# JinfengX/PointCloudPDF

Measured on AMD Instinct MI355X. Metric: points/sec fwd+bwd (PT-v1 Seg50 + PDF U-decoder, 100k-pt scenes), higher is better.
Workload: dtype f32

## Files before the change

include/pdfops.h:

```cpp
#ifndef PDFOPS_H
#define PDFOPS_H

#ifdef __cplusplus
extern "C" {
#endif

#define PDF_OK 0
#define PDF_ERR_BAD_ARG (-1)
#define PDF_ERR_NSAMPLE (-2)
#define PDF_ERR_UNSUPPORTED (-3)

#define PDF_ABI_VERSION 7
int pdf_abi_version(void);
const char *pdf_build_info(void);
int pdf_dist_fma_mode(void);
#define PDF_MMA_F32 0
#define PDF_MMA_F16 1
#define PDF_MMA_BF16 2

int pdf_knn_query(int m, int nsample, const float *xyz, const float *new_xyz,
                  const int *offset, const int *new_offset, int b,
                  int *idx, float *dist2, void *stream);

long pdf_knn_workspace_bytes(int b, int n, int m);
// ... 69 lines not shown
                      const float *new_xyz, const int *idx, float *output, void *stream);
int pdf_group_backward(int m, int nsample, int c, int with_xyz, const float *grad_output, const int *idx,
                       float *grad_feat, void *stream);

int pdf_interpolation_weights(int n, int k, const float *dist2, float *weight, void *stream);

int pdf_pt_layer_supported(int nsample, int c);
long pdf_pt_layer_partial_floats(int n, int nsample, int c);
int pdf_pt_layer_forward(int n, int nsample, int c, const float *xq, const float *xk, const float *xv,
                         const float *p, const int *idx, const float *const *weights,
                         const float *const *bn_params, float *const *bn_buffers, int training, float eps,
                         float momentum, float *bn, float *saved, float *H, float *partial, float *out,
                         int storage_bf16, const int *order, void *stream);
int pdf_pt_layer_forward_m(int n, int nsample, int c, const float *xq, const float *xk, const float *xv,
                           const float *p, const int *idx, const float *const *weights,
                           const float *const *bn_params, float *const *bn_buffers, int training, float eps,
                           float momentum, float *bn, float *saved, float *H, float *partial, float *out,
                           int storage_bf16, const int *order, const double *moments, int *out_stat_rows, void *stream);

long pdf_pt_layer_bwd_partial_floats(int n, int nsample, int c);
long pdf_pt_layer_bwd_sums_floats(int c);
int pdf_pt_layer_backward(int n, int nsample, int c, const float *xq, const float *xk, const float *xv,
                          const float *p, const int *idx, const float *const *weights, const float *bn,
                          const float *saved, const float *H, const float *gout, float *gxq, float *gxk,
                          float *gxv, float *G2, float *G3, float *Wsm, float *GR, const int *inv_off, const int *inv_entry,
                          int entry_base, float *partial, float *sums, int storage_bf16, const int *order, const double *moments,
                          void *stream);

int pdf_bn_supported(int c);
long pdf_bn_partial_floats(long n, int c);
int pdf_bn_act_forward(long n, int c, const float *x, const float *res, const float *gamma, const float *beta,
                       float *running_mean, float *running_var, int training, float eps, float momentum, int relu,
                       float *coef, float *partial, float *y, void *stream);
int pdf_bn_act_backward(long n, int c, const float *gy, const float *x, const float *res, const float *coef,
                        int training, int relu, float *partial, float *sums, float *gx, float *gres, void *stream);
int pdf_bn_coef(long n, int c, const float *x, const float *gamma, const float *beta, float *running_mean,
                float *running_var, int training, float eps, float momentum, float *coef, float *partial, void *stream);
int pdf_bn_apply(long n, int c, const float *x, const float *res, const float *coef, int relu, float *y, void *stream);

long pdf_rowlin_partial_floats(long n, int o);
int pdf_rowlin_partial_rows(long n, int k, int o);
int pdf_rowlin_forward(long n, int k, int o, const float *x, long ldx, const float *w, int transpose_w,
                       const float *bias, const float *scale, const float *shift, int relu, float *y, long ldy,
                       int accumulate, float *partial, int mma_input, void *stream);
long pdf_rowlin_wgrad_ws_floats(long n, int k, int o, int ng);
int pdf_rowlin_wgrad(long n, int k, int o, const float *g, long ldg, const float *x, long ldx,
                     const float *scale, const float *shift, int relu, float *dw, float *db, float *ws, int mma_input, void *stream);
int pdf_bn_coef_from_partial(const float *partial, int rows, long n, int c, const float *gamma, const float *beta,
                             float *running_mean, float *running_var, float eps, float momentum, float *coef, void *stream);

int pdf_rowlin_multi(long n, int k, int o, int nin, int nout, const float *const *x, long ldx, const float *const *w,
                     int transpose_w, const float *const *bias, const float *scale, const float *shift, int relu,
                     float *const *y, long ldy, int accumulate, int mma_input, void *stream);
int pdf_rowlin_wgrad_multi(long n, int k, int o, int ng, const float *const *g, long ldg, const float *x, long ldx,
                           const float *scale, const float *shift, int relu, float *const *dw, float *const *db, float *ws, int mma_input, void *stream);
int pdf_rowlin_wgrad_group(long n, int k, int o, int ng, const float *const *g, long ldg, const float *const *x, long ldx,
                           const float *const *scale, const float *const *shift, const int *relu, float *const *dw,
                           float *const *db, float *ws, int mma_input, void *stream);

int pdf_kpconv_supported(int kp, int cin);
int pdf_kpconv_gather(int n, int m, int kp, int cin, const float *query, const float *support, const int *neighbors, const float *x,
                      const float *k_points, float extent, float *weighted, void *stream);
int pdf_kpconv_scatter(int n, int m, int kp, int cin, const float *query, const float *support, const int *neighbors,
                       const float *grad_weighted, const float *k_points, float extent, float *grad_x, void *stream);
int pdf_rowlin_dgrad_bstats(long n, int k, int o, int nin, const float *const *x, long ldx, const float *const *w, float *y, long ldy,
                            const float *bx, long ldb, const float *bcoef, int brelu, float *partial, int *partial_rows,
                            int mma_input, void *stream);
int pdf_rowlin_forward_bn(long n, int k, int o, const float *x, long ldx, const float *w, const float *bias, const float *scale,
                          const float *shift, int relu, float *y, long ldy, float *partial, const float *gamma, const float *beta,
                          float *running_mean, float *running_var, float eps, float momentum, float *coef, int mma_input, void *stream);
int pdf_bn_act_backward_presummed(long n, int c, const float *gy, const float *x, const float *coef, int training, int relu,
                                  const float *partial, int partial_rows, float *sums, float *gx, void *stream);

int pdf_bn_coef_eval_or_partial(const float *partial, int rows, long n, int c, const float *gamma, const float *beta,
                                float *running_mean, float *running_var, int training, float eps, float momentum,
                                float *coef, void *stream);
int pdf_block_pre_forward(long n, int c, void *const *p, int training, float eps, float momentum, int mma_input, void *stream);
int pdf_block_pre_backward(long n, int c, void *const *p, int training, int mma_input, void *stream);
int pdf_block_post_forward(long n, int c, void *const *p, int training, float eps, float momentum, int mma_input, void *stream);
int pdf_block_post_backward(long n, int c, void *const *p, int training, int mma_input, void *stream);
int pdf_bottleneck_forward(long n, int nsample, int c, void *const *p, int training, float eps, float momentum, int storage_bf16, int mma_input, void *stream);
int pdf_bottleneck_backward(long n, int nsample, int c, void *const *p, int training, int entry_base, int storage_bf16, int mma_input, void *stream);
int pdf_linbn_forward(long n, int k, int o, void *const *p, int training, int relu, float eps, float momentum, int mma_input, void *stream);
int pdf_linbn_backward(long n, int k, int o, void *const *p, int training, int relu, int mma_input, void *stream);

int pdf_rowlin_forward_roww(long n, int k, int o, const float *x, long ldx, const float *w, int transpose_w, float *y, long ldy,
                            int accumulate, const float *roww, long rws, int mma_input, void *stream);
int pdf_rowlin_wgrad_roww(long n, int k, int o, const float *g, long ldg, const float *x, long ldx, float *dw, const float *roww,
                          long rws, float *ws, int mma_input, void *stream);
int pdf_bn_bwd_sums(long n, int c, const float *gy, const float *x, const float *coef, int relu, float *partial, float *sums,
                    void *stream);

int pdf_td_supported(int nsample, int cin, int cout);
int pdf_td_tables(long m, int b, const float *p_src, const float *p_new, const int *idx, const int *new_offset, float *rel4, float *Z,
                  float *scene_sums, long n, const int *inv_off, const int *inv_entry, int entry_base,
                  void *stream);
long pdf_td_gram_floats(int cin);
long pdf_td_fwd_scratch_floats(long n, int cin);
long pdf_td_bwd_scratch_floats(long m, int cin, int cout);
int pdf_td_forward(long n, long m, int cin, int cout, void *const *p, int training, float eps, float momentum, int mma_input, void *stream);
int pdf_td_backward(long n, long m, int cin, int cout, void *const *p, int entry_base, int mma_input, void *stream);

int pdf_seg_sum_rows(long n, int c, const float *src, const int *inv_off, const int *inv_entry, int entry_base, float scale, float *out,
                     void *stream);
int pdf_seg_sum_rows_own(long n, int c, int nsample, const float *src, const int *inv_off, const int *inv_entry, int entry_base, float scale,
                         const int *order, float *out, float *out_own, void *stream);
// ... 184 lines not shown
```

pointcloudpdf_amd/_native.py:

```python
import ctypes
import os
import threading

import torch

_HERE = os.path.dirname(os.path.abspath(__file__))
DIST_FMA = int(os.environ.get("PDFOPS_DIST_FMA", "0") or 0)
if DIST_FMA not in (0, 1, 2):
    raise RuntimeError(f"PDFOPS_DIST_FMA={DIST_FMA}: expected 0 (as written), 1 or 2 (csrc/pdfops_common.h)")


def library_path(dist_fma=0):
    return os.path.join(_HERE, "lib", "libpdfops.so" if not dist_fma else f"libpdfops_fma{int(dist_fma)}.so")


LIB_PATH = library_path(DIST_FMA)
ABI_VERSION = 7

c_int = ctypes.c_int
c_long = ctypes.c_long
c_void_p = ctypes.c_void_p
c_float = ctypes.c_float
c_double = ctypes.c_double

# ... 598 lines not shown
        self.CopySeg = CopySeg
        lib.pdf_stage_copy.restype = c_int
        lib.pdf_stage_copy.argtypes = [c_int, c_void_p, c_void_p]
        lib.pdf_scene_morton_keys.restype = c_int
        lib.pdf_scene_morton_keys.argtypes = [c_long, c_int, c_void_p, c_void_p, c_void_p, c_void_p, c_void_p]
        lib.pdf_sgd_chunk.restype = c_int
        lib.pdf_sgd_chunk.argtypes = []
        lib.pdf_sgd_step.restype = c_int
        lib.pdf_sgd_step.argtypes = [c_int, c_void_p, c_void_p, ctypes.c_float, ctypes.c_float, ctypes.c_float, c_void_p, c_void_p]
        lib.pdf_grad_unscale.restype = c_int
        lib.pdf_grad_unscale.argtypes = [c_int, c_void_p, c_void_p, c_void_p, c_void_p, c_void_p]
        lib.pdf_scaler_update.restype = c_int
        lib.pdf_scaler_update.argtypes = [c_void_p, c_void_p, c_void_p, c_void_p, ctypes.c_float, ctypes.c_float, c_int, c_void_p]
        lib.pdf_adam_step.restype = c_int
        lib.pdf_adam_step.argtypes = [c_int, c_int, c_void_p, c_void_p, ctypes.c_double, ctypes.c_double, ctypes.c_double, ctypes.c_double,
                                      ctypes.c_double, c_int, c_void_p, c_void_p]
        lib.pdf_adam_grad_unscale.restype = c_int
        lib.pdf_adam_grad_unscale.argtypes = [c_int, c_void_p, c_void_p, c_void_p, c_void_p, c_void_p]
        lib.pdf_linbn_forward.restype = c_int
        lib.pdf_linbn_forward.argtypes = [c_long, c_int, c_int, c_void_p, c_int, c_int, ctypes.c_float, ctypes.c_float, c_int, c_void_p]
        lib.pdf_linbn_backward.restype = c_int
        lib.pdf_linbn_backward.argtypes = [c_long, c_int, c_int, c_void_p, c_int, c_int, c_int, c_void_p]
        lib.pdf_bottleneck_forward.restype = c_int
        lib.pdf_bottleneck_forward.argtypes = [c_long, c_int, c_int, c_void_p, c_int, ctypes.c_float, ctypes.c_float, c_int, c_int, c_void_p]
        lib.pdf_bottleneck_backward.restype = c_int
        lib.pdf_bottleneck_backward.argtypes = [c_long, c_int, c_int, c_void_p, c_int, c_int, c_int, c_int, c_void_p]
        for nm in ("pre_backward", "post_backward"):
            f = getattr(lib, "pdf_block_" + nm)
            f.restype = c_int
            f.argtypes = [c_long, c_int, c_void_p, c_int, c_int, c_void_p]
        lib.pdf_rowlin_multi.restype = c_int
        lib.pdf_rowlin_multi.argtypes = [c_long, c_int, c_int, c_int, c_int, c_void_p, c_long, c_void_p, c_int, c_void_p, c_void_p, c_void_p,
                                         c_int, c_void_p, c_long, c_int, c_int, c_void_p]
        lib.pdf_kpconv_supported.restype = c_int
        lib.pdf_kpconv_supported.argtypes = [c_int, c_int]
        for nm in ("pdf_kpconv_gather", "pdf_kpconv_scatter"):
            f = getattr(lib, nm)
            f.restype = c_int
            f.argtypes = [c_int, c_int, c_int, c_int, c_void_p, c_void_p, c_void_p, c_void_p, c_void_p, ctypes.c_float, c_void_p, c_void_p]
        lib.pdf_rowlin_wgrad_group.restype = c_int
        lib.pdf_rowlin_wgrad_group.argtypes = [c_long, c_int, c_int, c_int, c_void_p, c_long, c_void_p, c_long, c_void_p, c_void_p, c_void_p,
                                               c_void_p, c_void_p, c_void_p, c_int, c_void_p]
        lib.pdf_rowlin_wgrad_multi.restype = c_int
        lib.pdf_rowlin_wgrad_multi.argtypes = [c_long, c_int, c_int, c_int, c_void_p, c_long, c_void_p, c_long, c_void_p, c_void_p, c_int,
                                               c_void_p, c_void_p, c_void_p, c_int, c_void_p]
        lib.pdf_rowlin_wgrad_ws_floats.restype = c_long
        lib.pdf_rowlin_wgrad_ws_floats.argtypes = [c_long, c_int, c_int, c_int]
        lib.pdf_rowlin_dgrad_bstats.restype = c_int
        lib.pdf_rowlin_dgrad_bstats.argtypes = [c_long, c_int, c_int, c_int, c_void_p, c_long, c_void_p, c_void_p, c_long, c_void_p, c_long,
                                                c_void_p, c_int, c_void_p, ctypes.POINTER(c_int), c_int, c_void_p]
        lib.pdf_bn_act_backward_presummed.restype = c_int
        lib.pdf_bn_act_backward_presummed.argtypes = [c_long, c_int, c_void_p, c_void_p, c_void_p, c_int, c_int, c_void_p, c_int, c_void_p,
                                                      c_void_p, c_void_p]
        lib.pdf_rowlin_partial_floats.restype = c_long
        lib.pdf_rowlin_partial_floats.argtypes = [c_long, c_int]
        lib.pdf_rowlin_partial_rows.restype = c_int
        lib.pdf_rowlin_partial_rows.argtypes = [c_long, c_int, c_int]
        lib.pdf_rowlin_forward.restype = c_int
        lib.pdf_rowlin_forward.argtypes = [c_long, c_int, c_int, c_void_p, c_long, c_void_p, c_int, c_void_p, c_void_p, c_void_p,
                                           c_int, c_void_p, c_long, c_int, c_void_p, c_int, c_void_p]
        lib.pdf_rowlin_wgrad.restype = c_int
        lib.pdf_rowlin_wgrad.argtypes = [c_long, c_int, c_int, c_void_p, c_long, c_void_p, c_long, c_void_p, c_void_p, c_int,
                                         c_void_p, c_void_p, c_void_p, c_int, c_void_p]
        lib.pdf_bn_coef_from_partial.restype = c_int
        lib.pdf_bn_coef_from_partial.argtypes = [c_void_p, c_int, c_long, c_int, c_void_p, c_void_p, c_void_p, c_void_p,
                                                 ctypes.c_float, ctypes.c_float, c_void_p, c_void_p]
        lib.pdf_bn_coef.restype = c_int
        lib.pdf_bn_coef.argtypes = [c_long, c_int, c_void_p, c_void_p, c_void_p, c_void_p, c_void_p, c_int, ctypes.c_float,
                                    ctypes.c_float, c_void_p, c_void_p, c_void_p]
        lib.pdf_bn_apply.restype = c_int
        lib.pdf_bn_apply.argtypes = [c_long, c_int, c_void_p, c_void_p, c_void_p, c_int, c_void_p, c_void_p]
        lib.pdf_bn_supported.restype = c_int
        lib.pdf_bn_supported.argtypes = [c_int]
        lib.pdf_bn_partial_floats.restype = c_long
        lib.pdf_bn_partial_floats.argtypes = [c_long, c_int]
        lib.pdf_bn_act_forward.restype = c_int
        lib.pdf_bn_act_forward.argtypes = [c_long, c_int] + [c_void_p] * 6 + [c_int, ctypes.c_float, ctypes.c_float, c_int] + [c_void_p] * 4
        lib.pdf_bn_act_backward.restype = c_int
        lib.pdf_bn_act_backward.argtypes = [c_long, c_int] + [c_void_p] * 4 + [c_int, c_int] + [c_void_p] * 5
        lib.pdf_pt_layer_supported.restype = c_int
        lib.pdf_pt_layer_supported.argtypes = [c_int, c_int]
        for fn in (lib.pdf_pt_layer_partial_floats, lib.pdf_pt_layer_bwd_partial_floats):
            fn.restype = c_long
            fn.argtypes = [c_int, c_int, c_int]
        lib.pdf_pt_layer_bwd_sums_floats.restype = c_long
        lib.pdf_pt_layer_bwd_sums_floats.argtypes = [c_int]
        lib.pdf_pt_layer_forward.restype = c_int
        lib.pdf_pt_layer_forward.argtypes = [c_int, c_int, c_int] + [c_void_p] * 8 + [c_int, ctypes.c_float, ctypes.c_float] + [c_void_p] * 5 + [c_int, c_void_p, c_void_p]
        lib.pdf_knn_grid_build.restype = c_int
        lib.pdf_knn_grid_build.argtypes = [c_int, c_void_p, c_void_p, c_int, c_void_p, c_long, c_void_p]
        lib.pdf_knn_query_grid.restype = c_int
        lib.pdf_knn_query_grid.argtypes = [c_int, c_int, c_int, c_void_p, c_void_p, c_void_p, c_void_p, c_int, c_void_p, c_void_p, c_void_p, c_long, c_void_p]
        lib.pdf_pt_layer_backward.restype = c_int
        lib.pdf_pt_layer_backward.argtypes = [c_int, c_int, c_int] + [c_void_p] * 19 + [c_int] + [c_void_p] * 2 + [c_int, c_void_p, c_void_p, c_void_p]
        self.fps_mode = os.environ.get("PDFOPS_FPS", "bucketed")
        self.knn_mode = os.environ.get("PDFOPS_KNN", "grid")
        lib.pdf_knn_workspace_bytes.restype = c_long
        lib.pdf_knn_workspace_bytes.argtypes = [c_int, c_int, c_int]
        lib.pdf_graph_forest_workspace_bytes.restype = c_long
        lib.pdf_region_grow_list_points.restype = c_long
        lib.pdf_region_grow_list_points.argtypes = []
        lib.pdf_graph_forest_workspace_bytes.argtypes = [c_long, c_long, c_long]
        lib.pdf_knn_grid_supported.restype = c_int
        lib.pdf_knn_grid_supported.argtypes = [c_int]
        lib.pdf_knn_query_ws.restype = c_int
        lib.pdf_knn_query_ws.argtypes = [c_int, c_int, c_int] + [c_void_p] * 4 + [c_int] + [c_void_p] * 3 + [c_long, c_void_p]
# ... 965 lines not shown
```

pointcloudpdf_amd/csrc/rowlin.hip:

```cpp
#include "pdfops_common.h"
#include <cstdlib>

namespace rl {

typedef float f32x16 __attribute__((ext_vector_type(16)));
constexpr int BM = 128, BN = 64, BK = 32, LDT = 33;

struct FwdArgs {
    long N;
    int K, O;
    const float *X; long ldx;
    const float *W; long wso, wsk;
    const float *bias;
    const float *scale, *shift;
    int relu;
    float *Y; long ldy;
    int accumulate;
    float *partial;
};

template <bool PRE, bool STATS>
__global__ __launch_bounds__(256) void k_rowlin(FwdArgs a) {
    __shared__ float xs[BM * LDT];
    __shared__ float ws[BN * LDT];
// ... 112 lines not shown
            g[u] = (r < re && ov) ? a.G[r * a.ldg + oc] : 0.f;
            float v = 0.f;
            if (r < re && cv) {
                v = a.X[r * a.ldx + cc];
                if (PRE) { v = v * sc + sh; if (a.relu) v = fmaxf(v, 0.f); }
            }
            x[u] = v;
        }
#pragma unroll
        for (int u = 0; u < 4; ++u) {
            acc = __builtin_amdgcn_mfma_f32_32x32x2f32(g[u], x[u], acc, 0, 0, 0);
            gsum += g[u];
        }
    }
    __shared__ float comb[4][1024 + 32];
#pragma unroll
    for (int r = 0; r < 16; ++r) {
        const int i = (r & 3) + 8 * (r >> 2) + 4 * (lane >> 5);
        comb[wave][i * 32 + ch] = acc[r];
    }
    gsum += __shfl_xor(gsum, 32, 64);
    if (lane < 32) comb[wave][1024 + ch] = gsum;
    __syncthreads();
    const size_t sidx = blockIdx.x, nsl = gridDim.x;
    float *slab = a.slab + ((size_t)blockIdx.y * nsl + sidx) * 1024;
#pragma unroll
    for (int e = threadIdx.x; e < 1024; e += 256) slab[e] = ((comb[0][e] + comb[1][e]) + comb[2][e]) + comb[3][e];
    if (a.db && c0 == 0 && threadIdx.x < 32)
        a.bslab[((size_t)(o0 / 32) * nsl + sidx) * 32 + threadIdx.x] =
            ((comb[0][1024 + threadIdx.x] + comb[1][1024 + threadIdx.x]) + comb[2][1024 + threadIdx.x]) + comb[3][1024 + threadIdx.x];
}

}

namespace rl2 {
int try_forward(long n, int k, int o, int nin, int nout, const float *const *x, long ldx, const float *const *w, int transpose_w,
                const float *const *bias, const float *scale, const float *shift, int relu, float *const *y, long ldy,
                int accumulate, float *partial, int mma, hipStream_t s, const float *roww = nullptr, long rws = 0, const float *bx = nullptr,
                long ldb = 0, const float *bcoef = nullptr, int brelu = 0, int *partial_rows = nullptr, long ldw = 0, void *handoff = nullptr);
long stats_rows_floats(long n, int o);
int try_wgrad(long n, int k, int o, int ng, const float *const *g, long ldg, const float *x, long ldx, const float *scale,
              const float *shift, int relu, float *const *dw, float *const *db, float *ws, int mma, hipStream_t s, const float *roww = nullptr, long rws = 0);
long wgrad_ws_floats(long n, int k, int o, int ng);
constexpr int WG_MAXG = 5;
struct RArgs {
    const float *slab, *bslab;
    float *dW[WG_MAXG], *db[WG_MAXG];
    int B, tiles_k, tiles, otiles, split, K, O;
};
int try_wgrad_group(long n, int k, int o, int ng, const float *const *g, long ldg, const float *const *x, long ldx, const float *const *scale,
                    const float *const *shift, const int *relu, float *const *dw, float *const *db, float *ws, int mma, hipStream_t s);
void launch_slab_reduce(const RArgs &a, int ng, bool any_bias, hipStream_t s);
int stats_rows(long n);
}

static inline void tiled_wg_plan(long n, int k, int o, int *blocks_oc, long *split, long *rows_per_block) {
    *blocks_oc = ((o + 31) / 32) * ((k + 31) / 32);
    long sp = (2048 + *blocks_oc - 1) / *blocks_oc;
    const long max_split = (n + 255) / 256;
    if (sp > max_split) sp = max_split;
    if (sp < 1) sp = 1;
    *rows_per_block = ((n + sp - 1) / sp + 31) / 32 * 32;
    *split = (n + *rows_per_block - 1) / *rows_per_block;
}

static inline bool rowlin_streams(int k, int o) {
    return (k == 32 || k == 64 || k == 128 || k == 256 || k == 512) && o % 16 == 0 && getenv("PDFOPS_ROWLIN_TILED") == nullptr;
}

extern "C" int pdf_rowlin_partial_rows(long n, int k, int o) {
    return rowlin_streams(k, o) ? rl2::stats_rows(n) : (int)((n + rl::BM - 1) / rl::BM);
}
extern "C" long pdf_rowlin_partial_floats(long n, int o) {
    const long a = (n + rl::BM - 1) / rl::BM * 2 * (long)o, b = rl2::stats_rows_floats(n, o);
    return (a > b ? a : b) + (long)PDF_HO_FLOATS;
}

extern "C" int pdf_rowlin_forward(long n, int k, int o, const float *x, long ldx, const float *w, int transpose_w,
                                  const float *bias, const float *scale, const float *shift, int relu, float *y, long ldy,
                                  int accumulate, float *partial, int mma_input, void *stream) {
    if (mma_input < 0 || mma_input > 2) return PDF_ERR_BAD_ARG;
    if (n < 1 || k < 1 || o < 1 || !x || !w || !y || ldx < k || ldy < o) return PDF_ERR_BAD_ARG;
    if (rowlin_streams(k, o)) {
        if (rl2::try_forward(n, k, o, 1, 1, &x, ldx, &w, transpose_w, &bias, scale, shift, relu, &y, ldy, accumulate, partial,
                             mma_input, static_cast<hipStream_t>(stream)))
            return pdf_launch_status();
        if (partial) return PDF_ERR_BAD_ARG;
    }
    if (!transpose_w && !partial && !scale && k == 1024 && rowlin_streams(512, o) && !(ldx & 3) && !(ldy & 3)) {
        const float *xs[2] = {x, x + 512}, *ws[2] = {w, w + 512};
        if (rl2::try_forward(n, 512, o, 2, 1, xs, ldx, ws, 0, &bias, nullptr, nullptr, 0, &y, ldy, accumulate, nullptr, mma_input, static_cast<hipStream_t>(stream),
                             nullptr, 0, nullptr, 0, nullptr, 0, nullptr, k))
            return pdf_launch_status();
    }
    rl::FwdArgs a;
    a.N = n; a.K = k; a.O = o; a.X = x; a.ldx = ldx; a.W = w;
    a.wso = transpose_w ? 1 : k; a.wsk = transpose_w ? o : 1;
    a.bias = bias; a.scale = scale; a.shift = shift; a.relu = relu; a.Y = y; a.ldy = ldy; a.accumulate = accumulate;
    a.partial = partial;
    const dim3 grid((unsigned)((n + rl::BM - 1) / rl::BM), (unsigned)((o + rl::BN - 1) / rl::BN));
    hipStream_t s = static_cast<hipStream_t>(stream);
    const bool pre = scale != nullptr, stats = partial != nullptr;
    if (pre && stats) rl::k_rowlin<true, true><<<grid, 256, 0, s>>>(a);
    else if (pre) rl::k_rowlin<true, false><<<grid, 256, 0, s>>>(a);
    else if (stats) rl::k_rowlin<false, true><<<grid, 256, 0, s>>>(a);
    else rl::k_rowlin<false, false><<<grid, 256, 0, s>>>(a);
    return pdf_launch_status();
}

extern "C" long pdf_rowlin_wgrad_ws_floats(long n, int k, int o, int ng) {
    if (n < 1 || k < 1 || o < 1 || ng < 1) return 0;
    int blocks_oc; long split, rpb;
    tiled_wg_plan(n, k, o, &blocks_oc, &split, &rpb);
    const long tiled = (long)blocks_oc * split * 4 * 1024 + (long)((o + 31) / 32) * split * 4 * 32;
    const long streaming = rowlin_streams(k, o) ? rl2::wgrad_ws_floats(n, k, o, ng) : 0;
    return tiled > streaming ? tiled : streaming;
}

extern "C" int pdf_bn_coef_from_partial(const float *partial, int rows, long n, int c, const float *gamma, const float *beta,
                                        float *running_mean, float *running_var, float eps, float momentum, float *coef, void *stream);

extern "C" int pdf_rowlin_forward_bn(long n, int k, int o, const float *x, long ldx, const float *w, const float *bias, const float *scale,
                                     const float *shift, int relu, float *y, long ldy, float *partial, const float *gamma, const float *beta,
                                     float *running_mean, float *running_var, float eps, float momentum, float *coef, int mma_input, void *stream) {
// ... 125 lines not shown
```

pointcloudpdf_amd/csrc/rowlin2_impl.h:

```cpp
#pragma once
#include "pdfops_common.h"
#include <algorithm>
#include <cstdlib>

namespace rl2 {

typedef float f32x4 __attribute__((ext_vector_type(4)));

typedef _Float16 h16x4 __attribute__((ext_vector_type(4)));
typedef __bf16 b16x4 __attribute__((ext_vector_type(4)));
typedef short s16x4 __attribute__((ext_vector_type(4)));
template <int MP> struct Mma;
template <> struct Mma<0> {
    typedef f32x4 frag;
    static __device__ __forceinline__ frag cvt(f32x4 v) { return v; }
};
template <> struct Mma<1> {
    typedef h16x4 frag;
    static __device__ __forceinline__ frag cvt(f32x4 v) { return __builtin_convertvector(v, h16x4); }
    static __device__ __forceinline__ f32x4 mma(frag a, frag b, f32x4 acc) { return __builtin_amdgcn_mfma_f32_16x16x16f16(a, b, acc, 0, 0, 0); }
};
template <> struct Mma<2> {
    typedef s16x4 frag;
    static __device__ __forceinline__ frag cvt(f32x4 v) { return __builtin_bit_cast(s16x4, __builtin_convertvector(v, b16x4)); }
// ... 126 lines not shown
                            for (int ob = 0; ob < NOB; ++ob)
                                acc[ob] = __builtin_amdgcn_mfma_f32_16x16x4f32(Wr[in][ob][j][c], x4[c], acc[ob], 0, 0, 0);
                    } else {
                        const wfrag xh = Mma<MP>::cvt(x4);
#pragma unroll
                        for (int ob = 0; ob < NOB; ++ob) acc[ob] = Mma<MP>::mma(Wr[in][ob][j], xh, acc[ob]);
                    }
                }
            }
        }
#pragma unroll
        for (int ob = 0; ob < NOB; ++ob) {
            f32x4 v = acc[ob];
            if (a.roww) v *= a.roww[(valid ? n : 0) * a.rws];
            v += bias4[ob];
            float *dst = a.Y[outi[ob]] + (valid ? n : 0) * a.ldy + colb[ob] + 4 * kq;
            if (a.accumulate && valid) v += *reinterpret_cast<const f32x4 *>(dst);
            if (valid) *reinterpret_cast<f32x4 *>(dst) = v;
            if (ST == 1 && valid) { s4[ob] += v; ss4[ob] += v * v; }
            if (ST == 2) {
                const f32x4 x4 = *reinterpret_cast<const f32x4 *>(a.bx + (valid ? n : 0) * a.ldb + colb[ob] + 4 * kq);
                const f32x4 sc = *reinterpret_cast<const f32x4 *>(&bco[0][ob * 16 + 4 * kq]);
                const f32x4 sh = *reinterpret_cast<const f32x4 *>(&bco[ST == 2 ? 1 : 0][ob * 16 + 4 * kq]);
                const f32x4 mu = *reinterpret_cast<const f32x4 *>(&bco[ST == 2 ? 2 : 0][ob * 16 + 4 * kq]);
                const f32x4 pre = x4 * sc + sh;
                f32x4 gm;
#pragma unroll
                for (int c = 0; c < 4; ++c) gm[c] = (valid && (!a.brelu || pre[c] > 0.f)) ? v[c] : 0.f;
                s4[ob] += gm;
                ss4[ob] += gm * (x4 - mu);
            }
        }
    }
    if (STATS) {
        __shared__ float red[4][2][NOB * 16];
#pragma unroll
        for (int ob = 0; ob < NOB; ++ob)
#pragma unroll
            for (int r = 0; r < 4; ++r) {
                float s = s4[ob][r], ss = ss4[ob][r];
#pragma unroll
                for (int m = 1; m < 16; m <<= 1) { s += __shfl_xor(s, m, 64); ss += __shfl_xor(ss, m, 64); }
                if (li == 0) { red[wave][0][ob * 16 + 4 * kq + r] = s; red[wave][1][ob * 16 + 4 * kq + r] = ss; }
            }
        __syncthreads();
        const int t = threadIdx.x;
        if (t < NOB * 16) {
            float *row = a.partial + (size_t)blockIdx.x * 2 * a.O;
            row[gcol0 + t] = red[0][0][t] + red[1][0][t] + red[2][0][t] + red[3][0][t];
            const float ss = red[0][1][t] + red[1][1][t] + red[2][1][t] + red[3][1][t];
            row[a.O + gcol0 + t] = ST == 2 ? ss * a.bcoef[3 * (long)a.O + gcol0 + t] : ss;
        }
    }
}

constexpr int WG_MAXG = 5;
struct WArgs {
    long N;
    int K, O;
    const float *G[WG_MAXG]; long ldg;
    const float *X; long ldx;
    const float *scale, *shift; int relu;
    int per_z; const float *Xz[WG_MAXG]; const float *scalez[WG_MAXG], *shiftz[WG_MAXG]; int reluz[WG_MAXG];
    float *dW[WG_MAXG], *db[WG_MAXG];
    long rows_per_block;
    const float *roww; long rws;
    float *slab;
    float *bslab;
};

template <int VW> struct Vec;
template <> struct Vec<2> { typedef float type __attribute__((ext_vector_type(2))); };
template <> struct Vec<4> { typedef float type __attribute__((ext_vector_type(4))); };

template <int VW, bool PRE, bool RW, int MP>
__global__ __launch_bounds__(256) void k_wg(WArgs a) {
    typedef typename Vec<VW>::type vec;
    constexpr int B = 16 * VW;
    __shared__ float red[4][B * B];
    __shared__ float redb[4][B];
    const int lane = threadIdx.x & 63, wave = threadIdx.x >> 6;
    const int li = lane & 15, nq = lane >> 4;
    const int nkb = a.K / B;
    const int ob = (blockIdx.y / nkb) * B, kb = (blockIdx.y % nkb) * B;
    const float *G = a.G[blockIdx.z];
    const float *X = (PRE && a.per_z) ? a.Xz[blockIdx.z] : a.X;
    vec sc, sh;
    bool relu = a.relu != 0;
    if (PRE) {
        const float *scp = a.per_z ? a.scalez[blockIdx.z] : a.scale, *shp = a.per_z ? a.shiftz[blockIdx.z] : a.shift;
        if (a.per_z) relu = scp != nullptr && a.reluz[blockIdx.z] != 0;
        if (scp) {
            sc = *reinterpret_cast<const vec *>(scp + kb + VW * li);
            sh = *reinterpret_cast<const vec *>(shp + kb + VW * li);
        } else {
#pragma unroll
            for (int c = 0; c < VW; ++c) { sc[c] = 1.f; sh[c] = 0.f; }
        }
    }
    const float relu_lo = relu ? 0.f : -INFINITY;
    f32x4 acc[VW][VW];
    float gsum[VW];
#pragma unroll
    for (int c = 0; c < VW; ++c) {
        gsum[c] = 0.f;
#pragma unroll
// ... 151 lines not shown
static inline bool aligned16(const void *p) { return (reinterpret_cast<uintptr_t>(p) & 15) == 0; }

template <int K, int NOB, int NIN, int MP>
static int launch_fwd(const FwdArgs &a, int nslabs, hipStream_t s) {
    const bool pre = a.scale != nullptr, stats = a.partial != nullptr, bst = stats && a.bx != nullptr;
    static const int total = [] { const char *v = getenv("PDFOPS_RL_BLOCKS"); const int x = v ? atoi(v) : 0; return x > 0 ? x : 512; }();
    int gx = fwd_row_blocks(a.N);
    if (!stats || bst) gx = std::max(1, std::min(gx, std::max(8, total / std::max(nslabs, 1))));
    const dim3 grid((unsigned)gx, (unsigned)nslabs);
    if (bst) {
        k_fwd<K, NOB, NIN, false, 2, MP><<<grid, 256, 0, s>>>(a);
    } else if (NIN == 1 && stats) {
        if (pre) k_fwd<K, NOB, 1, true, 1, MP><<<grid, 256, 0, s>>>(a);
        else k_fwd<K, NOB, 1, false, 1, MP><<<grid, 256, 0, s>>>(a);
    } else {
        if (pre) k_fwd<K, NOB, NIN, true, 0, MP><<<grid, 256, 0, s>>>(a);
        else k_fwd<K, NOB, NIN, false, 0, MP><<<grid, 256, 0, s>>>(a);
    }
    return gx;
}

#ifdef RL2_MAIN_TU
long stats_rows_floats(long n, int o) { return (long)fwd_row_blocks(n) * 2 * o; }
#endif

template <int MP>
int try_forward_mp(long n, int k, int o, int nin, int nout, const float *const *x, long ldx, const float *const *w, int transpose_w,
                   const float *const *bias, const float *scale, const float *shift, int relu, float *const *y, long ldy,
                   int accumulate, float *partial, hipStream_t s, const float *roww, long rws, const float *bx, long ldb, const float *bcoef,
                   int brelu, int *partial_rows, long ldw, void *handoff) {
    if (nin < 1 || nout < 1 || (nin > 1 && nout > 1) || nin > 3 || nout > 3) return 0;
    if (nin == 2 && (scale || bx)) return 0;
    if (partial && !bx && (nin != 1 || nout != 1)) return 0;
    if (bx && (!partial || nout != 1 || scale || !bcoef || (ldb & 3) || !aligned16(bx) || !aligned16(bcoef))) return 0;
    if ((ldx & 3) || (ldy & 3) || (o & 15)) return 0;
    for (int i = 0; i < (nin > 1 ? nin : nout); ++i) if (!aligned16(w[i])) return 0;
    if (scale && (!aligned16(scale) || !aligned16(shift))) return 0;
    for (int i = 0; i < nin; ++i) if (!aligned16(x[i])) return 0;
    for (int i = 0; i < nout; ++i) if (!aligned16(y[i])) return 0;
    FwdArgs a;
    a.N = n; a.O = o; a.ldx = ldx; a.ldy = ldy; a.scale = scale; a.shift = shift; a.relu = relu; a.accumulate = accumulate;
    a.partial = partial; a.roww = roww; a.rws = rws;
    a.bx = bx; a.ldb = ldb; a.bcoef = bcoef; a.brelu = brelu;
    a.ho_gran = static_cast<unsigned long long *>(handoff);
    a.ho_sync = handoff ? reinterpret_cast<unsigned *>(a.ho_gran + 2 * (size_t)o) : nullptr;
    a.wso = transpose_w ? 1 : (ldw ? ldw : k); a.wsk = transpose_w ? o : 1;
    for (int i = 0; i < 3; ++i) {
        a.X[i] = i < nin ? x[i] : nullptr;
        a.W[i] = i < (nin > 1 ? nin : nout) ? w[i] : nullptr;
        a.bias[i] = (bias && i < nout) ? bias[i] : nullptr;
        a.Y[i] = i < nout ? y[i] : nullptr;
    }
    const int cols = o * nout;
#define PDF_RL2(K_, NOB_, NIN_) do { if (cols % (NOB_ * 16) == 0) { \
        const int r_ = launch_fwd<K_, NOB_, NIN_, MP>(a, cols / (NOB_ * 16), s); \
        if (partial_rows) *partial_rows = r_; \
        return 1; } } while (0)
    if (nin == 1) {
        switch (k) {
        case 32: if (!partial) PDF_RL2(32, 6, 1); PDF_RL2(32, 2, 1); PDF_RL2(32, 1, 1); break;
        case 64: PDF_RL2(64, 4, 1); PDF_RL2(64, 1, 1); break;
        case 128: if (!bx) PDF_RL2(128, 4, 1); else PDF_RL2(128, 2, 1); PDF_RL2(128, 1, 1); break;
        case 256: PDF_RL2(256, 2, 1); PDF_RL2(256, 1, 1); break;
        case 512: PDF_RL2(512, 1, 1); break;
        default: break;
        }
    } else if (nin == 2) {
        if (k == 512) PDF_RL2(512, 1, 2);
    } else if (nin == 3) {
        switch (k) {
        case 32: PDF_RL2(32, 2, 3); break;
        case 64: PDF_RL2(64, 2, 3); break;
        case 128: PDF_RL2(128, 1, 3); break;
        case 256: PDF_RL2(256, 1, 3); break;
        default: break;
        }
    }
#undef PDF_RL2
    return 0;
}

template <int MP>
int try_wgrad_mp(long n, int k, int o, int ng, const float *const *g, long ldg, const float *x, long ldx, const float *scale,
                 const float *shift, int relu, float *const *dw, float *const *db, float *ws, hipStream_t s, const float *roww, long rws) {
    if (ng < 1 || ng > 3 || !ws) return 0;
    const WgPlan p = wg_plan(n, k, o, ng);
    const int vw = p.vw;
    if (!vw) return 0;
    if ((ldg % vw) || (ldx % vw) || !aligned16(x)) return 0;
    if (scale && (!aligned16(scale) || !aligned16(shift))) return 0;
    for (int i = 0; i < ng; ++i) if (!aligned16(g[i])) return 0;
    WArgs a;
    a.N = n; a.K = k; a.O = o; a.ldg = ldg; a.X = x; a.ldx = ldx; a.scale = scale; a.shift = shift; a.relu = relu; a.roww = roww; a.rws = rws;
    a.per_z = 0;
    bool any_bias = false;
    for (int i = 0; i < WG_MAXG; ++i) {
        a.G[i] = i < ng ? g[i] : nullptr; a.dW[i] = i < ng ? dw[i] : nullptr; a.db[i] = (db && i < ng) ? db[i] : nullptr;
        a.Xz[i] = nullptr; a.scalez[i] = a.shiftz[i] = nullptr; a.reluz[i] = 0;
        any_bias = any_bias || a.db[i] != nullptr;
    }
    const int b = p.b;
    a.rows_per_block = p.rows_per_block;
    a.slab = ws;
    a.bslab = ws + (size_t)p.nblk * p.split * b * b;
    const dim3 grid((unsigned)p.split, (unsigned)((o / b) * (k / b)), (unsigned)ng);
#define PDF_WG(VW_) do { \
        if (roww) { if (scale) k_wg<VW_, true, true, MP><<<grid, 256, 0, s>>>(a); else k_wg<VW_, false, true, MP><<<grid, 256, 0, s>>>(a); } \
        else      { if (scale) k_wg<VW_, true, false, MP><<<grid, 256, 0, s>>>(a); else k_wg<VW_, false, false, MP><<<grid, 256, 0, s>>>(a); } } while (0)
    if (vw == 4) PDF_WG(4); else PDF_WG(2);
#undef PDF_WG
    RArgs r;
    r.slab = a.slab; r.bslab = a.bslab; r.B = b; r.tiles_k = k / b; r.tiles = (o / b) * (k / b); r.otiles = o / b; r.split = (int)p.split; r.K = k; r.O = o;
    for (int i = 0; i < WG_MAXG; ++i) { r.dW[i] = a.dW[i]; r.db[i] = a.db[i]; }
    launch_slab_reduce(r, ng, any_bias, s);
    return 1;
}

template <int MP>
int try_wgrad_group_mp(long n, int k, int o, int ng, const float *const *g, long ldg, const float *const *x, long ldx,
                       const float *const *scale, const float *const *shift, const int *relu, float *const *dw, float *const *db,
                       float *ws, hipStream_t s) {
    if (ng < 1 || ng > WG_MAXG || !ws) return 0;
    const WgPlan p = wg_plan(n, k, o, ng);
    const int vw = p.vw;
    if (!vw) return 0;
    if ((ldg % vw) || (ldx % vw)) return 0;
    for (int i = 0; i < ng; ++i) {
        if (!aligned16(g[i]) || !aligned16(x[i])) return 0;
        if (scale[i] && (!aligned16(scale[i]) || !aligned16(shift[i]))) return 0;
    }
    WArgs a;
    a.N = n; a.K = k; a.O = o; a.ldg = ldg; a.X = nullptr; a.ldx = ldx; a.scale = a.shift = nullptr; a.relu = 0; a.roww = nullptr; a.rws = 0;
    a.per_z = 1;
    bool any_bias = false;
    for (int i = 0; i < WG_MAXG; ++i) {
        const bool on = i < ng;
        a.G[i] = on ? g[i] : nullptr; a.Xz[i] = on ? x[i] : nullptr;
        a.scalez[i] = on ? scale[i] : nullptr; a.shiftz[i] = on ? shift[i] : nullptr; a.reluz[i] = on ? relu[i] : 0;
        a.dW[i] = on ? dw[i] : nullptr; a.db[i] = (on && db) ? db[i] : nullptr;
        any_bias = any_bias || a.db[i] != nullptr;
    }
    const int b = p.b;
    a.rows_per_block = p.rows_per_block;
    a.slab = ws;
    a.bslab = ws + (size_t)p.nblk * p.split * b * b;
    const dim3 grid((unsigned)p.split, (unsigned)((o / b) * (k / b)), (unsigned)ng);
    if (vw == 4) k_wg<4, true, false, MP><<<grid, 256, 0, s>>>(a); else k_wg<2, true, false, MP><<<grid, 256, 0, s>>>(a);
    RArgs r;
    r.slab = a.slab; r.bslab = a.bslab; r.B = b; r.tiles_k = k / b; r.tiles = (o / b) * (k / b); r.otiles = o / b; r.split = (int)p.split; r.K = k; r.O = o;
    for (int i = 0; i < WG_MAXG; ++i) { r.dW[i] = a.dW[i]; r.db[i] = a.db[i]; }
    launch_slab_reduce(r, ng, any_bias, s);
    return 1;
}

#ifdef RL2_MAIN_TU
int stats_rows(long n) { return fwd_row_blocks(n); }
#endif

}
```

Baseline: 13.49 million.

## Add LDS-tiled MFMA forward kernel for multi-input/multi-output row linears

Adds a new forward kernel that stages 64-row by 64-K chunks of X (and transposed W for the 3-input case) in shared memory, with register prefetch of the next chunk. It is used for K in {128, 256, 512} with (nin=1, nout=3) or (nin=3, nout=1), and includes optional pre-scale/ReLU and fused BN-backward stats. The aim is to reuse each X tile across several output column tiles instead of streaming it from global memory per column block. A grid-size threshold chooses a narrow or wide column-block layout. It costs extra LDS traffic and barriers, and it is enabled by default with an env opt-out.

After: 13.71 million (median of 6 runs). 1.6% higher.

```diff
diff --git a/include/pdfops.h b/include/pdfops.h
--- a/include/pdfops.h
+++ b/include/pdfops.h
@@ -145,6 +145,7 @@
 int pdf_rowlin_multi(long n, int k, int o, int nin, int nout, const float *const *x, long ldx, const float *const *w,
                      int transpose_w, const float *const *bias, const float *scale, const float *shift, int relu,
                      float *const *y, long ldy, int accumulate, int mma_input, void *stream);
+int pdf_rowlin_tiled_covers(long n, int k, int nin, int nout, int bstats);
 int pdf_rowlin_wgrad_multi(long n, int k, int o, int ng, const float *const *g, long ldg, const float *x, long ldx,
                            const float *scale, const float *shift, int relu, float *const *dw, float *const *db, float *ws, int mma_input, void *stream);
 int pdf_rowlin_wgrad_group(long n, int k, int o, int ng, const float *const *g, long ldg, const float *const *x, long ldx,
diff --git a/pointcloudpdf_amd/_native.py b/pointcloudpdf_amd/_native.py
--- a/pointcloudpdf_amd/_native.py
+++ b/pointcloudpdf_amd/_native.py
@@ -674,6 +674,8 @@
         lib.pdf_bn_act_backward_presummed.restype = c_int
         lib.pdf_bn_act_backward_presummed.argtypes = [c_long, c_int, c_void_p, c_void_p, c_void_p, c_int, c_int, c_void_p, c_int, c_void_p,
                                                       c_void_p, c_void_p]
+        lib.pdf_rowlin_tiled_covers.restype = c_int
+        lib.pdf_rowlin_tiled_covers.argtypes = [c_long, c_int, c_int, c_int, c_int]
         lib.pdf_rowlin_partial_floats.restype = c_long
         lib.pdf_rowlin_partial_floats.argtypes = [c_long, c_int]
         lib.pdf_rowlin_partial_rows.restype = c_int
diff --git a/pointcloudpdf_amd/csrc/rowlin.hip b/pointcloudpdf_amd/csrc/rowlin.hip
--- a/pointcloudpdf_amd/csrc/rowlin.hip
+++ b/pointcloudpdf_amd/csrc/rowlin.hip
@@ -188,6 +188,7 @@
                     const float *const *shift, const int *relu, float *const *dw, float *const *db, float *ws, int mma, hipStream_t s);
 void launch_slab_reduce(const RArgs &a, int ng, bool any_bias, hipStream_t s);
 int stats_rows(long n);
+int tiled_covers_probe(long n, int k, int nin, int nout, int bstats);
 }
 
 static inline void tiled_wg_plan(long n, int k, int o, int *blocks_oc, long *split, long *rows_per_block) {
@@ -206,6 +207,9 @@
 
 extern "C" int pdf_rowlin_partial_rows(long n, int k, int o) {
     return rowlin_streams(k, o) ? rl2::stats_rows(n) : (int)((n + rl::BM - 1) / rl::BM);
+}
+extern "C" int pdf_rowlin_tiled_covers(long n, int k, int nin, int nout, int bstats) {
+    return rowlin_streams(k, k) ? rl2::tiled_covers_probe(n, k, nin, nout, bstats) : 0;
 }
 extern "C" long pdf_rowlin_partial_floats(long n, int o) {
     const long a = (n + rl::BM - 1) / rl::BM * 2 * (long)o, b = rl2::stats_rows_floats(n, o);
diff --git a/pointcloudpdf_amd/csrc/rowlin2_impl.h b/pointcloudpdf_amd/csrc/rowlin2_impl.h
--- a/pointcloudpdf_amd/csrc/rowlin2_impl.h
+++ b/pointcloudpdf_amd/csrc/rowlin2_impl.h
@@ -202,6 +202,192 @@
             row[a.O + gcol0 + t] = ST == 2 ? ss * a.bcoef[3 * (long)a.O + gcol0 + t] : ss;
         }
     }
+}
+
+constexpr int TL_ROWS = 64, TL_KC = 64, TL_LD = TL_KC + 4;
+
+template <int K, int WR, int NIN, bool PRE, int ST, int MP>
+__global__ __launch_bounds__(256) void k_fwd_tiled(FwdArgs a) {
+    typedef typename Mma<MP>::frag wfrag;
+    constexpr bool TW = NIN > 1;
+    constexpr int WC = 4 / WR, RT = 4 / WR;
+    constexpr int CB = 16 * WC, WLD = CB + 4;
+    constexpr int NCH = K / TL_KC, NS = NIN * NCH, NJ = TL_KC / 16;
+    constexpr int CPR = CB / 4, RPP = 256 / CPR, NWP = TL_KC / RPP;
+    __shared__ __attribute__((aligned(16))) float xs[TL_ROWS * TL_LD];
+    __shared__ __attribute__((aligned(16))) float wsm[TW ? TL_KC * WLD : 4];
+    const int lane = threadIdx.x & 63, wave = threadIdx.x >> 6;
+    const int li = lane & 15, kq = lane >> 4;
+    const int wr = wave / WC, wc = wave % WC;
+    const long row0 = (long)blockIdx.x * TL_ROWS;
+    const int gcol0 = blockIdx.y * CB;
+    const int outi = (gcol0 + wc * 16) / a.O, colb = gcol0 + wc * 16 - outi * a.O;
+    const int sx_c = 4 * (threadIdx.x & 15), sx_r = threadIdx.x >> 4;
+    const int sw_c = 4 * (threadIdx.x % CPR), sw_r = threadIdx.x / CPR;
+    long xoff[4];
+#pragma unroll
+    for (int i = 0; i < 4; ++i) { const long n = row0 + sx_r + 16 * i; xoff[i] = (n < a.N ? n : 0) * a.ldx + sx_c; }
+    const float *wrow = nullptr;
+    if (!TW) wrow = (outi == 0 ? a.W[0] : (outi == 1 ? a.W[1] : a.W[2])) + (long)(colb + li) * a.wso + 4 * kq;
+    const float relu_lo = a.relu ? 0.f : -INFINITY;
+    f32x4 xpf[4], scpf, shpf, wpf[TW ? NWP : NJ], wcur[TW ? 1 : NJ];
+    auto prefetch = [&](int s) {
+        const int in = s / NCH, kc0 = (s - in * NCH) * TL_KC;
+        const float *X = in == 0 ? a.X[0] : (in == 1 ? a.X[1] : a.X[2]);
+#pragma unroll
+        for (int i = 0; i < 4; ++i) xpf[i] = *reinterpret_cast<const f32x4 *>(X + xoff[i] + kc0);
+        if (PRE) {
+            scpf = *reinterpret_cast<const f32x4 *>(a.scale + kc0 + sx_c);
+            shpf = *reinterpret_cast<const f32x4 *>(a.shift + kc0 + sx_c);
+        }
+        if (TW) {
+            const float *W = in == 0 ? a.W[0] : (in == 1 ? a.W[1] : a.W[2]);
+#pragma unroll
+            for (int i = 0; i < NWP; ++i) wpf[i] = *reinterpret_cast<const f32x4 *>(W + (long)(kc0 + sw_r + RPP * i) * a.wsk + gcol0 + sw_c);
+        } else {
+#pragma unroll
+            for (int j = 0; j < NJ; ++j) wpf[j] = *reinterpret_cast<const f32x4 *>(wrow + kc0 + 16 * j);
+        }
+    };
+    f32x4 acc[RT];
+#pragma unroll
+    for (int t = 0; t < RT; ++t) acc[t] = f32x4{0.f, 0.f, 0.f, 0.f};
+    prefetch(0);
+#pragma unroll 1
+    for (int s = 0; s < NS; ++s) {
+        __syncthreads();
+#pragma unroll
+        for (int i = 0; i < 4; ++i) {
+            f32x4 x4 = xpf[i];
+            if (PRE) {
+                x4 = x4 * scpf + shpf;
+#pragma unroll
+                for (int c = 0; c < 4; ++c) x4[c] = fmaxf(x4[c], relu_lo);
+            }
+            *reinterpret_cast<f32x4 *>(&xs[(sx_r + 16 * i) * TL_LD + sx_c]) = x4;
+        }
+        if (TW) {
+#pragma unroll
+            for (int i = 0; i < NWP; ++i) *reinterpret_cast<f32x4 *>(&wsm[TW ? (sw_r + RPP * i) * WLD + sw_c : 0]) = wpf[i];
+        } else {
+#pragma unroll
+            for (int j = 0; j < NJ; ++j) wcur[TW ? 0 : j] = wpf[j];
+        }
+        __syncthreads();
+        if (s + 1 < NS) prefetch(s + 1);
+#pragma unroll
+        for (int j = 0; j < NJ; ++j) {
+            f32x4 a4, x4[RT];
+            if (TW) {
+#pragma unroll
+                for (int c = 0; c < 4; ++c) a4[c] = wsm[TW ? (16 * j + 4 * kq + c) * WLD + wc * 16 + li : 0];
+            } else {
+                a4 = wcur[TW ? 0 : j];
+            }
+#pragma unroll
+            for (int t = 0; t < RT; ++t) x4[t] = *reinterpret_cast<const f32x4 *>(&xs[(16 * (wr * RT + t) + li) * TL_LD + 16 * j + 4 * kq]);
+            if constexpr (MP == 0) {
+#pragma unroll
+                for (int c = 0; c < 4; ++c)
+#pragma unroll
+                    for (int t = 0; t < RT; ++t) acc[t] = __builtin_amdgcn_mfma_f32_16x16x4f32(a4[c], x4[t][c], acc[t], 0, 0, 0);
+            } else {
+                const wfrag ah = Mma<MP>::cvt(a4);
+#pragma unroll
+                for (int t = 0; t < RT; ++t) acc[t] = Mma<MP>::mma(ah, Mma<MP>::cvt(x4[t]), acc[t]);
+            }
+        }
+    }
+    const float *b = NIN > 1 ? a.bias[0] : (outi == 0 ? a.bias[0] : (outi == 1 ? a.bias[1] : a.bias[2]));
+    float *Y = outi == 0 ? a.Y[0] : (outi == 1 ? a.Y[1] : a.Y[2]);
+    const int col = colb + 4 * kq;
+    f32x4 bias4 = f32x4{0.f, 0.f, 0.f, 0.f};
+    if (b) bias4 = *reinterpret_cast<const f32x4 *>(b + col);
+    f32x4 bsc, bsh, bmu, s4 = f32x4{0.f, 0.f, 0.f, 0.f}, ss4 = f32x4{0.f, 0.f, 0.f, 0.f};
+    if (ST == 2) {
+        bsc = *reinterpret_cast<const f32x4 *>(a.bcoef + col);
+        bsh = *reinterpret_cast<const f32x4 *>(a.bcoef + (long)a.O + col);
+        bmu = *reinterpret_cast<const f32x4 *>(a.bcoef + 2 * (long)a.O + col);
+    }
+#pragma unroll
+    for (int t = 0; t < RT; ++t) {
+        const long n = row0 + 16 * (wr * RT + t) + li;
+        const bool valid = n < a.N;
+        const long nn = valid ? n : 0;
+        f32x4 v = acc[t];
+        if (a.roww) v *= a.roww[nn * a.rws];
+        v += bias4;
+        float *dst = Y + nn * a.ldy + col;
+        if (a.accumulate && valid) v += *reinterpret_cast<const f32x4 *>(dst);
+        if (valid) *reinterpret_cast<f32x4 *>(dst) = v;
+        if (ST == 2) {
+            const f32x4 x4 = *reinterpret_cast<const f32x4 *>(a.bx + nn * a.ldb + col);
+            const f32x4 pre = x4 * bsc + bsh;
+            f32x4 gm;
+#pragma unroll
+            for (int c = 0; c < 4; ++c) gm[c] = (valid && (!a.brelu || pre[c] > 0.f)) ? v[c] : 0.f;
+            s4 += gm;
+            ss4 += gm * (x4 - bmu);
+        }
+    }
+    if (ST == 2) {
+        __shared__ float red[WR][2][CB];
+        float *row = a.partial + (size_t)blockIdx.x * 2 * a.O;
+#pragma unroll
+        for (int r = 0; r < 4; ++r) {
+            float sv = s4[r], ssv = ss4[r];
+#pragma unroll
+            for (int m = 1; m < 16; m <<= 1) { sv += __shfl_xor(sv, m, 64); ssv += __shfl_xor(ssv, m, 64); }
+            if (li == 0) {
+                if (WR == 1) { row[col + r] = sv; row[a.O + col + r] = ssv * a.bcoef[3 * (long)a.O + col + r]; }
+                else { red[wr][0][wc * 16 + 4 * kq + r] = sv; red[wr][1][wc * 16 + 4 * kq + r] = ssv; }
+            }
+        }
+        if (WR > 1) {
+            __syncthreads();
+            const int t = threadIdx.x;
+            if (t < CB) {
+                float sv = red[0][0][t], ssv = red[0][1][t];
+#pragma unroll
+                for (int g = 1; g < WR; ++g) { sv += red[g][0][t]; ssv += red[g][1][t]; }
+                row[gcol0 + t] = sv;
+                row[a.O + gcol0 + t] = ssv * a.bcoef[3 * (long)a.O + gcol0 + t];
+            }
+        }
+    }
+}
+
+static inline bool tiled_enabled() {
+    static const bool on = [] { const char *v = getenv("PDFOPS_RL_TILED"); return !(v && atoi(v) == 0); }();
+    return on;
+}
+static inline long tiled_max_rows(int k) {
+    switch (k) {
+    case 128: return (long)FWD_CAP * TL_ROWS;
+    case 256: return (long)FWD_CAP * TL_ROWS;
+    case 512: return (long)FWD_CAP * TL_ROWS;
+    default: return 0;
+    }
+}
+static inline bool tiled_covers(long n, int k, int nin, int nout, int bstats) {
+    if (!tiled_enabled() || n < 1 || n > tiled_max_rows(k)) return false;
+    if ((n + TL_ROWS - 1) / TL_ROWS > FWD_CAP) return false;
+    return (nin == 1 && nout == 3 && !bstats) || (nin == 3 && nout == 1);
+}
+
+template <int K, int NIN, int MP>
+static int launch_fwd_tiled(const FwdArgs &a, int cols, hipStream_t s) {
+    static const int split = [] { const char *v = getenv("PDFOPS_RL_TILED_SPLIT"); return v ? atoi(v) : 256; }();
+    const int gx = (int)((a.N + TL_ROWS - 1) / TL_ROWS);
+    const bool narrow = (long)gx * (cols / 64) < split;
+    const dim3 grid((unsigned)gx, (unsigned)(cols / (narrow ? 32 : 64)));
+    const bool pre = a.scale != nullptr, bst = a.bx != nullptr;
+#define PDF_TL(WR_) do { \
+        if constexpr (NIN == 1) { if (pre) k_fwd_tiled<K, WR_, 1, true, 0, MP><<<grid, 256, 0, s>>>(a); else k_fwd_tiled<K, WR_, 1, false, 0, MP><<<grid, 256, 0, s>>>(a); } \
+        else { if (bst) k_fwd_tiled<K, WR_, NIN, false, 2, MP><<<grid, 256, 0, s>>>(a); else k_fwd_tiled<K, WR_, NIN, false, 0, MP><<<grid, 256, 0, s>>>(a); } } while (0)
+    if (narrow) PDF_TL(2); else PDF_TL(1);
+#undef PDF_TL
+    return gx;
 }
 
 constexpr int WG_MAXG = 5;
@@ -459,6 +645,13 @@
         a.Y[i] = i < nout ? y[i] : nullptr;
     }
     const int cols = o * nout;
+    if (tiled_covers(n, k, nin, nout, bx != nullptr) && o % 64 == 0 && !handoff && (nin == 1 ? (!transpose_w && !partial) : (transpose_w && !scale && (!partial || bx)))) {
+        int r_ = 0;
+        if (nin == 1) r_ = k == 128 ? launch_fwd_tiled<128, 1, MP>(a, cols, s) : (k == 256 ? launch_fwd_tiled<256, 1, MP>(a, cols, s) : launch_fwd_tiled<512, 1, MP>(a, cols, s));
+        else r_ = k == 128 ? launch_fwd_tiled<128, 3, MP>(a, cols, s) : (k == 256 ? launch_fwd_tiled<256, 3, MP>(a, cols, s) : launch_fwd_tiled<512, 3, MP>(a, cols, s));
+        if (partial_rows) *partial_rows = r_;
+        return 1;
+    }
 #define PDF_RL2(K_, NOB_, NIN_) do { if (cols % (NOB_ * 16) == 0) { \
         const int r_ = launch_fwd<K_, NOB_, NIN_, MP>(a, cols / (NOB_ * 16), s); \
         if (partial_rows) *partial_rows = r_; \
@@ -562,6 +755,7 @@
 
 #ifdef RL2_MAIN_TU
 int stats_rows(long n) { return fwd_row_blocks(n); }
+int tiled_covers_probe(long n, int k, int nin, int nout, int bstats) { return tiled_covers(n, k, nin, nout, bstats) ? 1 : 0; }
 #endif
 
 }
```
